# kentchen831213/-Distributed-Machine-Learning-System

Hardware: AMD Instinct MI355X
Metric: images/sec (whole node) + p50 query latency, ResNet18 bs=400 at 1/2/4/8 GPU (higher is better)
Workload: dtype fp32; 1 GPU; model=resnet18, global_batch=400, image_hw=224, batch_per_gpu=400, parallelism=dp1, graph=True, fp32_impl=split, dry_run=False

## Files before the change

### -distributed-machine-learning-system_amd/csrc/bindings.cpp

```cpp
#include <ATen/hip/HIPContext.h>
#include <torch/extension.h>

#include <mutex>

#include "kernels.h"
#include "launch_util.h"
#include "runtime/jpeg_entropy.h"

using namespace idunno;

static hipStream_t cur_stream() { return at::hip::getCurrentHIPStream().stream(); }

static void check_launch(const char* what) {
  const hipError_t e = hipGetLastError();
  TORCH_CHECK(e == hipSuccess, what, ": HIP launch failed: ", hipGetErrorString(e));
}

static torch::Tensor zero_buffer(const torch::Device& dev) {
  static std::mutex mu;
  static std::vector<torch::Tensor>* bufs = new std::vector<torch::Tensor>(64);
  const int i = dev.index() < 0 ? 0 : dev.index();
  TORCH_CHECK(i < 64, "device index out of range");
  std::lock_guard<std::mutex> lk(mu);
  auto& b = (*bufs)[i];
// ... 590 lines not shown
  TORCH_CHECK(conv3x3_band_launch(reinterpret_cast<const half_t*>(x.data_ptr()), C,
                                  reinterpret_cast<const half_t*>(w.data_ptr()), bias.data_ptr<float>(), rp, Cout,
                                  y.data_ptr(), Cout, false, B, H, W, C, Cout, relu ? 1 : 0, 1.0f, nullptr,
                                  (int)max_grid, 0, cur_stream(), true),
              "band conv: tensor too large for 32-bit buffer offsets");
  check_launch("conv3x3_band (fp16)");
  return y;
}

torch::Tensor conv2d_split(torch::Tensor x, torch::Tensor w, torch::Tensor bias, c10::optional<torch::Tensor> res,
                           int64_t KH, int64_t KW, int64_t stride, int64_t pad, bool relu, double acc_scale,
                           bool out_f32, int64_t tile, c10::optional<torch::Tensor> out, int64_t ksplit,
                           int64_t route) {
  return conv2d_split_impl(x, w, bias, res, KH, KW, stride, pad, relu, acc_scale, out_f32, tile, out, 0, false, 1.0,
                           ksplit, route);
}

torch::Tensor conv2d_split_dual(torch::Tensor x, torch::Tensor w, torch::Tensor bias, int64_t KH, int64_t KW,
                                int64_t stride, int64_t pad, bool relu, double acc_scale, double acc_scale2,
                                int64_t nsplit, bool center_only, int64_t tile) {
  TORCH_CHECK(nsplit > 0, "dual conv needs nsplit > 0");
  return conv2d_split_impl(x, w, bias, c10::nullopt, KH, KW, stride, pad, relu, acc_scale, false, tile,
                           c10::nullopt, nsplit, center_only, acc_scale2, 1, 0);
}

torch::Tensor linear_split(torch::Tensor x, torch::Tensor w, torch::Tensor bias, double acc_scale, bool relu,
                           bool out_f32, int64_t splits, int64_t tile) {
  CHECK_DEV(x);
  CHECK_DEV(w);
  CHECK_DEV(bias);
  CHECK_CONTIG(x);
  CHECK_CONTIG(w);
  CHECK_CONTIG(bias);
  CHECK_DT(x, torch::kHalf);
  CHECK_DT(w, torch::kHalf);
  CHECK_DT(bias, torch::kFloat);
  TORCH_CHECK(x.dim() == 2 && w.dim() == 2 && bias.dim() == 1, "bad ranks");
  TORCH_CHECK(w.device() == x.device() && bias.device() == x.device(), "operands on different devices");
  const int64_t M = x.size(0), K2 = x.size(1), N = w.size(0);
  TORCH_CHECK(w.size(1) == K2 && bias.size(0) == N, "shape mismatch");
  TORCH_CHECK(out_f32 ? N % 4 == 0 : N % 32 == 0, "N must be a multiple of 4 (fp32 out) / 32 (split out)");
  TORCH_CHECK(splits >= 1 && splits <= 16 && K2 % (64 * splits) == 0, "K must split into multiples of 32");
  TORCH_CHECK(splits * M * N < (1L << 31) && M * K2 < (1L << 31), "too large for int32 indexing");
  auto part = torch::empty({splits, M, N}, x.options().dtype(torch::kFloat));
  auto y = out_f32 ? torch::empty({M, N}, x.options().dtype(torch::kFloat))
                   : torch::empty({M, 2 * N}, x.options().dtype(torch::kHalf));
// ... 1066 lines not shown
  m.def("conv1x1_dual_ok", &conv1x1_dual_ok, "whether conv1x1_dual supports (K1, K2, Cout, M)");
  m.def("conv1x1_fused_next", &conv1x1_fused_next, "bottleneck tail + next block's reduce 1x1 in one pass (fp16)",
        py::arg("x1"), py::arg("x2"), py::arg("w"), py::arg("bias"), py::arg("res"), py::arg("w2"), py::arg("b2"),
        py::arg("stride"), py::arg("relu"));
  m.def("conv1x1_fused_next_ok", &conv1x1_fused_next_ok, "whether conv1x1_fused_next supports (K1, K2, N, N2, M)");
  m.def("conv1x1_dual_split", &conv1x1_dual_split, "split (fp32-accurate) form of conv1x1_dual", py::arg("x1"),
        py::arg("x2"), py::arg("w"), py::arg("bias"), py::arg("acc_scale"), py::arg("stride"), py::arg("relu"));
  m.def("conv1x1_dual_split_ok", &conv1x1_dual_split_ok, "whether conv1x1_dual_split supports (K1, K2, Cout, M)");
  m.def("conv2d_nhwc", &conv2d_nhwc, "implicit-GEMM MFMA conv + bias (+res) (+relu)", py::arg("x"), py::arg("w"),
        py::arg("bias"), py::arg("res"), py::arg("KH"), py::arg("KW"), py::arg("stride"), py::arg("pad"),
        py::arg("relu"), py::arg("out_f32") = false, py::arg("tile") = -1, py::arg("out") = py::none(),
        py::arg("ksplit") = -1, py::arg("route") = 0);
  m.def("linear_splitk", &linear_splitk, "FC layer with split-K partial GEMMs + combine", py::arg("x"),
        py::arg("w"), py::arg("bias"), py::arg("relu"), py::arg("out_f32"), py::arg("splits"), py::arg("tile") = -1);
  m.def("conv2d_split", &conv2d_split, "split-fp16 (fp32-accurate) conv: 3 f16 MFMAs per 32 channels",
        py::arg("x"), py::arg("w"), py::arg("bias"), py::arg("res"), py::arg("KH"), py::arg("KW"), py::arg("stride"),
        py::arg("pad"), py::arg("relu"), py::arg("acc_scale"), py::arg("out_f32") = false, py::arg("tile") = -1,
        py::arg("out") = py::none(), py::arg("ksplit") = -1, py::arg("route") = 0);
  m.def("conv2d_split_dual", &conv2d_split_dual,
        "two split convs of one input in one launch (downsample as the centre tap of the 3x3/s conv)",
        py::arg("x"), py::arg("w"), py::arg("bias"), py::arg("KH"), py::arg("KW"), py::arg("stride"), py::arg("pad"),
        py::arg("relu"), py::arg("acc_scale"), py::arg("acc_scale2"), py::arg("nsplit"), py::arg("center_only"),
        py::arg("tile") = -1);
  m.def("conv2d_pack3_split", &conv2d_pack3_split, "split-fp16 RGB stem conv on packed rows, fp32 out",
        py::arg("x3"), py::arg("w"), py::arg("bias"), py::arg("W"), py::arg("KH"), py::arg("KW"), py::arg("stride"),
        py::arg("pad"), py::arg("relu"), py::arg("acc_scale"), py::arg("tile") = -1);
  m.def("preprocess_pack3_split", &preprocess_pack3_split, "uint8 HWC -> split-fp16 packed-row stem input",
        py::arg("img"), py::arg("KW"), py::arg("stride"), py::arg("pad"), py::arg("start") = py::none(),
        py::arg("batch") = -1, py::arg("start_offset") = 0, py::arg("window") = -1, py::arg("sub") = 0);
  m.def("stem_u8_f16", &stem_u8_f16, "fp16 fused ResNet stem in exact-u8 form (pack_stem_split weights)",
        py::arg("img"), py::arg("w"), py::arg("bias"), py::arg("psum"), py::arg("acc_scale"), py::arg("start") = py::none(),
        py::arg("batch") = -1, py::arg("start_offset") = 0, py::arg("window") = -1, py::arg("sub") = 0);
  m.def("stem_split", &stem_split, "fp32-accurate fused split-fp16 ResNet stem (normalise+conv7x7/2+relu+maxpool)",
        py::arg("img"), py::arg("w"), py::arg("bias"), py::arg("psum"), py::arg("acc_scale"), py::arg("start") = py::none(),
        py::arg("batch") = -1, py::arg("start_offset") = 0, py::arg("window") = -1, py::arg("sub") = 0);
  m.def("linear_split", &linear_split, "fp32-accurate FC on split fp16, split-K in one launch + combine",
        py::arg("x"), py::arg("w"), py::arg("bias"), py::arg("acc_scale"), py::arg("relu"), py::arg("out_f32"),
        py::arg("splits"), py::arg("tile") = -1);
  m.def("conv3x3_band_split", &conv3x3_band_split,
        "band-staged split 3x3/s1/p1 conv (tile 70) with a persistent-grid cap (0: one workgroup per CU)",
        py::arg("x"), py::arg("w"), py::arg("bias"), py::arg("res") = py::none(), py::arg("relu") = true,
        py::arg("acc_scale") = 1.0, py::arg("out_f32") = false, py::arg("max_grid") = 0, py::arg("flags") = 0);
  m.def("conv3x3_band_f16", &conv3x3_band_f16,
        "band-staged fp16 3x3/s1/p1 conv (tile 70) with a persistent-grid cap (0: one workgroup per CU)",
        py::arg("x"), py::arg("w"), py::arg("bias"), py::arg("res"), py::arg("relu"), py::arg("max_grid") = 0);
  m.def("conv3x3_band_tiles", &conv3x3_band_tiles, "band conv tile count for (B, W, Cout)");
// ... 82 lines not shown
```

### -distributed-machine-learning-system_amd/csrc/kernels.h

```cpp
#pragma once
#include "common.h"

namespace idunno {

struct ConvArgs {
  const half_t* x;
  const half_t* w;
  const float* bias;
  const half_t* res;
  void* y;
  int B, H, W, C;
  int Ho, Wo, Cout, ldy;
  int KH, KW, stride, pad;
  int M;
  int nK;
  int cblk;
  int nsub;
  int Kpad;
  int relu;
  int tiles_n;
  int tiles_m;
  const void* zero;
  int ldx;
  int nc, wp, cpk;
  int ksplit;
  int kslice;
  long ysplit;
  float acc_scale;
  int* ovf;
  int nsplit_n;
  int center_only;
  float acc_scale2;
  int ldr;
  int kstage;
};

struct ConvF32Args {
  const float* x;
  const float* w;
  const float* bias;
  const float* res;
  float* y;
  int B, H, W, C;
  int Ho, Wo, Cout, ldy;
  int KH, KW, stride, pad;
  int M;
  int nK;
  int cblk;
  int nsub;
  int Kpad;
  int relu;
  int tiles_n, tiles_m;
  const void* zero;
  int ldx;
  int nc, wp, cpk;
  int ksplit;
  int kslice;
// ... 28 lines not shown
                                 long long sub, hipStream_t st);
void preprocess_pack3_f16_launch(const uint8_t* img, half_t* out, int B, int H, int W, int pad, int nc, int wp,
                                 const long long* start_idx, long long start_off, long long max_start,
                                 long long sub, hipStream_t st);
void preprocess_pack3_split_launch(const uint8_t* img, half_t* out, int B, int H, int W, int pad, int nc, int wp,
                                   const long long* start_idx, long long start_off, long long max_start,
                                   long long sub, hipStream_t st);
void preprocess_f32_launch(const uint8_t* img, float* out, long npix, const long long* start_idx,
                           long long start_off, long long max_start, long long sub, long pix_per_img,
                           hipStream_t st);
void maxpool_f32_launch(const float* x, float* y, int B, int H, int W, int C, int Ho, int Wo, int k, int s,
                        int pad, hipStream_t st);
void avgpool_f32_launch(const float* x, float* y, int B, int HW, int C, hipStream_t st);
void split_from_f32_launch(const float* x, half_t* y, long npix, int C, int* ovf, hipStream_t st);
void f32_from_split_launch(const half_t* x, float* y, long npix, int C, hipStream_t st);
void maxpool_split_launch(const void* x, bool in_split, half_t* y, int B, int H, int W, int C, int Ho, int Wo, int k,
                          int s, int pad, int* ovf, hipStream_t st);

void conv_igemm_launch(ConvArgs a, bool small, bool out_f32, int tile, hipStream_t st);
int conv_pick_tile(int M, int Cout);
bool conv_glds_launch(ConvArgs a, bool out_f32, int tile, hipStream_t st);
bool conv_glds_split_launch(ConvArgs a, bool out_f32, int tile, hipStream_t st);
int conv_glds_split_pick(int M, int Cout);
int conv_split_ksplit(int M, int Cout, int tile, int nk_total, int force, bool legacy = false);
bool conv1x1_small_m(long M);
void splitk_reduce_res_launch(const float* part, int S, long MN, int N, const float* bias, const half_t* res,
                              int ldr, int relu, void* y, int ldy, int fmt, int* ovf, hipStream_t st);
int conv_f16_ksplit(int M, int Cout, int tile, int nk_total, int force);
bool conv1x1_stream_supported(int C, int Cout, long M);
bool conv1x1_stream_launch(const half_t* x, const half_t* w, const float* bias, const half_t* res, half_t* y,
                           const void* zero, int M, int C, int Cout, int relu, int H, int W, int Wo, int HWo,
                           int stride, hipStream_t st);
bool conv1x1_stream_default(int C, int stride, long M);
bool conv1x1_stream_split_supported(int C, int Cout, long M);
bool conv1x1_stream_split_launch(const half_t* x, const half_t* w, const float* bias, const half_t* res, half_t* y,
                                 const void* zero, int M, int C, int Cout, int relu, float acc_scale, int* ovf, int H,
                                 int W, int Wo, int HWo, int stride, hipStream_t st);
bool conv1x1_dual_supported(int K1, int K2, int Cout, long M);
bool conv1x1_dual_launch(const half_t* x1, const half_t* x2, const half_t* w, const float* bias, half_t* y,
                         const void* zero, int M, int K1, int K2, int Cout, int relu, int H, int W, int Wo, int HWo,
                         int stride, hipStream_t st);
bool conv1x1_dual_split_supported(int K1, int K2, int Cout, long M);
bool conv1x1_dual_split_launch(const half_t* x1, const half_t* x2, const half_t* w, const float* bias, half_t* y,
                               const void* zero, int M, int K1, int K2, int Cout, int relu, float acc_scale, int* ovf,
                               int H, int W, int Wo, int HWo, int stride, hipStream_t st);
bool conv1x1_fused_next_supported(int K1, int K2, int N, int N2, long M);
// ... 81 lines not shown
```

### -distributed-machine-learning-system_amd/csrc/kernels/conv_glds.hip

```cpp
#include "../kernels.h"
#include "../launch_util.h"

namespace idunno {

typedef __attribute__((address_space(3))) void lds_void_t;
typedef __attribute__((address_space(1))) void glb_void_t;


template <int N>
__device__ __forceinline__ void wait_vmcnt() {
  static_assert(N >= 0 && N < 64, "vmcnt range");
  asm volatile("s_waitcnt vmcnt(%0)" ::"n"(N) : "memory");
}

template <int G, int NS>
__device__ __forceinline__ void wait_stages(int pending_stages) {
  if constexpr (NS >= 4) {
    if (pending_stages >= 2) { wait_vmcnt<2 * G>(); return; }
  }
  if constexpr (NS >= 3) {
    if (pending_stages >= 1) { wait_vmcnt<G>(); return; }
  }
  wait_vmcnt<0>();
}

template <int BN, int BM, int BK, int WN, int WM, int NS, bool HAS_RES, bool OUT_F32, bool P3 = false,
          bool SPLIT = false, bool KS = false>
__global__ void __launch_bounds__(64 * WN * WM, (BM % 64 != 0 && WN * WM == 8) ? 4 : 1)
conv_glds_kernel(const ConvArgs a) {
  static_assert(!SPLIT || BK == 64, "split stages are 32 channels x (hi, lo)");
  static_assert(!KS || (OUT_F32 && !HAS_RES && !P3), "split-K writes fp32 partials");
  constexpr int NW = WN * WM;
  constexpr int NT = 64 * NW;
  constexpr int TN = BN / WN, TM = BM / WM;
  constexpr int FN = TN / 16, FM = TM / 16;
  constexpr int CPR = BK / 8;
  constexpr int RB = BK * 2;
  constexpr int RPI = 64 / CPR;
  constexpr int BMD = (BM + RPI * NW - 1) / (RPI * NW) * (RPI * NW);
  constexpr int A_INS = BN / RPI, B_INS = BMD / RPI;
  static_assert(A_INS % NW == 0 && B_INS % NW == 0, "DMA instructions must split evenly over waves");
  constexpr int GA = A_INS / NW, GB = B_INS / NW, G = GA + GB;
  constexpr int A_BYTES = BN * RB, STAGE = (BN + BMD) * RB;
  static_assert(NS >= 2 && NS <= 4, "ring depth");
  static_assert(G * (NS - 2) < 64, "vmcnt immediate");

  extern __shared__ __attribute__((aligned(16))) char smem[];
  const int tid = threadIdx.x, lane = tid & 63;
  const int wave = __builtin_amdgcn_readfirstlane(tid >> 6);
  const int wn = wave / WM, wm = wave % WM;

  const int nwg = a.tiles_n * a.tiles_m;
  const int nsplit = a.ksplit > 1 ? a.ksplit : 1;
  const int lid_all = xcd_remap(blockIdx.x, nwg * nsplit);
// ... 50 lines not shown
    i_kh = a.KH / 2;
    i_kw = a.KW / 2;
    i_s = (i_kh * a.KW + i_kw) * a.cblk;
    nK = a.cblk;
  }
  if constexpr (KS) {
    i_s = split * a.kstage;
    i_cb = i_s % a.cblk;
    const int tap = i_s / a.cblk;
    i_kw = tap % a.KW;
    i_kh = tap / a.KW;
    nK = a.kstage;
  }
  constexpr uint32_t OOR = 0x80000000u;
  const auto w_rsrc = __builtin_amdgcn_make_buffer_rsrc((void*)win, 0, 0x7fffffff, 0x00020000);
  const auto x_rsrc = __builtin_amdgcn_make_buffer_rsrc((void*)xin, 0, 0x7fffffff, 0x00020000);
  uint32_t a_voff[GA], b_voff[GB];
#pragma unroll
  for (int j = 0; j < GA; ++j) {
    const int n = n0 + (wave + NW * j) * RPI + lrow;
    a_voff[j] = n < a.Cout ? (uint32_t)((n * a.Kpad + a_ch[j]) * 2) : OOR;
  }
  auto set_tap = [&]() {
#pragma unroll
    for (int j = 0; j < GB; ++j) {
      const int ih = b_ih0[j] + i_kh, iw = b_iw0[j] + i_kw;
      const bool ok = (unsigned)ih < (unsigned)a.H && (unsigned)iw < (unsigned)a.W;
      b_voff[j] = ok ? (uint32_t)((b_base[j] + (ih * a.W + iw) * ldx) * 2) : OOR;
    }
  };
  if constexpr (KS) {
    if (i_cb != 0) set_tap();
  }
  auto issue_buf = [&](int buf) {
    char* base = smem + buf * STAGE;
    if (i_cb == 0) set_tap();
    const int koff = i_s * BK * 2, coff = i_cb * BK * 2;
#pragma unroll
    for (int j = 0; j < GA; ++j)
      dma_buf16(w_rsrc, base + (wave + NW * j) * 1024, a_voff[j], koff);
#pragma unroll
    for (int j = 0; j < GB; ++j) {
      if constexpr (BMD != BM) {
        static_assert(BMD == BM || (NS == 2 && BM % RPI == 0), "skipped padding instructions need vmcnt(0) waits");
        if ((wave + NW * j) * RPI >= BM) continue;
      }
      dma_buf16(x_rsrc, base + A_BYTES + (wave + NW * j) * 1024, b_voff[j], coff);
    }
    ++i_s;
    if (++i_cb == a.cblk) {
      i_cb = 0;
      if (++i_kw == a.KW) {
        i_kw = 0;
        ++i_kh;
      }
    }
  };
  auto issue_glb = [&](int buf) {
    char* base = smem + buf * STAGE;
    const int koff = i_s * BK;
#pragma unroll
    for (int j = 0; j < GA; ++j) {
      const half_t* src = a_src[j] ? a_src[j] + koff : zero;
      __builtin_amdgcn_global_load_lds((glb_void_t*)src, (lds_void_t*)(base + (wave + NW * j) * 1024), 16, 0, 0);
    }
    const int coff = i_cb * BK;
#pragma unroll
    for (int j = 0; j < GB; ++j) {
      if constexpr (P3) {
        int q, poff = 0;
        if constexpr (SPLIT) {
          const int cc = b_ch[j] / 8;
          q = i_s * 4 + (cc & 3);
// ... 233 lines not shown
      if constexpr (OUT_F32) {
        *reinterpret_cast<float4v*>(static_cast<float*>(a.y) + (size_t)split * a.ysplit + (size_t)m * a.ldy + n) = v;
      } else if constexpr (SPLIT) {
        split_guard(a.ovf, v);
        half4v h, l;
        split_f16x4(v, h, l);
        const int q = lane >> 4;
        half_t* yp = static_cast<half_t*>(a.y) + (size_t)m * a.ldy + split_off_q(n - 4 * q, q);
        *reinterpret_cast<u32x4_sw*>(yp) = split_swap_out(h, l);
      } else {
        half4v o;
        o[0] = (half_t)v[0];
        o[1] = (half_t)v[1];
        o[2] = (half_t)v[2];
        o[3] = (half_t)v[3];
        *reinterpret_cast<half4v*>(static_cast<half_t*>(a.y) + (size_t)m * a.ldy + n) = o;
      }
    }
  }
}

static bool glds_fits(const ConvArgs& a) {
  const long xb = (long)a.B * a.H * a.W * (a.ldx ? a.ldx : a.C) * 2, wb = (long)a.Cout * a.Kpad * 2;
  return xb < (1L << 31) && wb < (1L << 31);
}

template <int BN, int BM, int BK, int WN, int WM, int NS, bool HAS_RES, bool OUT_F32, bool P3 = false,
          bool SPLIT = false, bool KS = false>
static void glds_cfg(ConvArgs a, hipStream_t st) {
  a.tiles_n = (a.Cout + BN - 1) / BN;
  a.tiles_m = (a.M + BM - 1) / BM;
  if (P3) {
    a.cblk = 1;
    const int cps = SPLIT ? BK / 16 : BK / 8;
    a.nK = (a.KH * a.cpk + cps - 1) / cps;
  } else {
    a.cblk = a.C / BK;
    a.nK = a.KH * a.KW * a.cblk;
  }
  const int grid = a.tiles_n * a.tiles_m * (a.ksplit > 1 ? a.ksplit : 1);
  constexpr int RPI_ = 64 / (BK / 8), NW_ = WN * WM;
  constexpr int BMD = (BM + RPI_ * NW_ - 1) / (RPI_ * NW_) * (RPI_ * NW_);
  const size_t lds = (size_t)NS * (BN + BMD) * BK * 2;
  auto kern = conv_glds_kernel<BN, BM, BK, WN, WM, NS, HAS_RES, OUT_F32, P3, SPLIT, KS>;
  ensure_lds_attr(reinterpret_cast<const void*>(kern), (int)lds);
  hipLaunchKernelGGL(kern, dim3(grid), dim3(64 * WN * WM), lds, st, a);
}

template <bool R, bool F>
static bool glds_dispatch(ConvArgs a, int tile, hipStream_t st) {
  switch (tile) {
    case 10: glds_cfg<128, 128, 64, 2, 2, 3, R, F>(a, st); return true;
    case 11: glds_cfg<128, 128, 32, 2, 2, 4, R, F>(a, st); return true;
    case 12: glds_cfg<64, 256, 64, 1, 4, 3, R, F>(a, st); return true;
    case 13: glds_cfg<64, 256, 32, 1, 4, 4, R, F>(a, st); return true;
    case 14: glds_cfg<128, 256, 64, 2, 4, 3, R, F>(a, st); return true;
    case 15: glds_cfg<64, 128, 64, 1, 4, 3, R, F>(a, st); return true;
    case 16: glds_cfg<128, 64, 64, 2, 2, 3, R, F>(a, st); return true;
    case 17: glds_cfg<256, 128, 64, 4, 2, 3, R, F>(a, st); return true;
    case 18: glds_cfg<128, 128, 32, 2, 2, 3, R, F>(a, st); return true;
    case 19: glds_cfg<128, 64, 32, 2, 2, 4, R, F>(a, st); return true;
    case 20: glds_cfg<64, 128, 32, 1, 4, 4, R, F>(a, st); return true;
    case 21: glds_cfg<256, 128, 32, 4, 2, 4, R, F>(a, st); return true;
    case 22: glds_cfg<128, 256, 32, 2, 4, 4, R, F>(a, st); return true;
    case 23: glds_cfg<64, 64, 64, 2, 2, 3, R, F>(a, st); return true;
    case 24: glds_cfg<128, 128, 64, 2, 4, 3, R, F>(a, st); return true;
    case 25: glds_cfg<256, 128, 64, 4, 2, 2, R, F>(a, st); return true;
// ... 39 lines not shown
}

template <bool R, bool F>
static bool glds_dispatch_split(ConvArgs a, int tile, hipStream_t st) {
  switch (tile) {
    case 26: glds_cfg<128, 128, 64, 2, 2, 2, R, F, false, true>(a, st); return true;
    case 27: glds_cfg<64, 128, 64, 1, 4, 2, R, F, false, true>(a, st); return true;
    case 34: glds_cfg<128, 64, 64, 2, 2, 2, R, F, false, true>(a, st); return true;
    case 36: glds_cfg<128, 128, 64, 2, 4, 2, R, F, false, true>(a, st); return true;
    case 38: glds_cfg<128, 64, 64, 2, 4, 2, R, F, false, true>(a, st); return true;
    case 42: glds_cfg<128, 160, 64, 4, 2, 2, R, F, false, true>(a, st); return true;
    default: return false;
  }
}

bool conv_glds_split_launch(ConvArgs a, bool out_f32, int tile, hipStream_t st) {
  if (!glds_fits(a)) return false;
  if (a.kstage > 0) return out_f32 && a.res == nullptr && glds_dispatch_ks<true>(a, tile, st);
  const bool res = a.res != nullptr;
  if (res) return out_f32 ? glds_dispatch_split<true, true>(a, tile, st) : glds_dispatch_split<true, false>(a, tile, st);
  return out_f32 ? glds_dispatch_split<false, true>(a, tile, st) : glds_dispatch_split<false, false>(a, tile, st);
}

static void ks_tile_dims(int tile, int& bn, int& bm) {
  switch (tile) {
    case 42: bn = 128; bm = 160; return;
    case 27: bn = 64; bm = 128; return;
    default: bn = 128; bm = 128; return;
  }
}
static int ksplit_rule(int force, int M, int Cout, int tile, int nk_total, long target_blocks, int min_stages) {
  if (tile != 27 && tile != 36 && tile != 42) return 1;
  if (force == 0 || force == 1) return 1;
  if (force > 1) return nk_total % force == 0 ? force : 1;
  if (nk_total < 2 * min_stages) return 1;
  int bn, bm;
  ks_tile_dims(tile, bn, bm);
  const long blocks = (long)((M + bm - 1) / bm) * ((Cout + bn - 1) / bn);
  int s = 1;
  while (s < 8 && blocks * s * 2 <= target_blocks && nk_total % (s * 2) == 0 && nk_total / (s * 2) >= min_stages)
    s *= 2;
  return s;
}
int conv_split_ksplit(int M, int Cout, int tile, int nk_total, int force, bool legacy) {
  if (legacy) return ksplit_rule(force, M, Cout, tile, nk_total, 2L * device_cu_count(), 4);
  return ksplit_rule(force, M, Cout, tile, nk_total, (long)device_cu_count(), 8);
}
int conv_f16_ksplit(int M, int Cout, int tile, int nk_total, int force) {
  return ksplit_rule(force, M, Cout, tile, nk_total, 2L * device_cu_count(), 4);
}

int conv_glds_split_pick(int M, int Cout) {
  if (Cout % 128 == 0) return M >= 50000 ? 36 : 42;
  return 27;
}

bool conv1x1_small_m(long M) { return M < 16384; }

bool conv_glds_split_p3_launch(ConvArgs a, int tile, hipStream_t st) {
  if (a.res != nullptr || a.cpk <= 0) return false;
  switch (tile) {
    case 23: glds_cfg<64, 64, 64, 2, 2, 3, false, true, true, true>(a, st); return true;
    case 27: glds_cfg<64, 128, 64, 1, 4, 2, false, true, true, true>(a, st); return true;
    case 33: glds_cfg<64, 256, 64, 1, 4, 2, false, true, true, true>(a, st); return true;
    case 35: glds_cfg<64, 64, 64, 2, 2, 2, false, true, true, true>(a, st); return true;
    case 37: glds_cfg<64, 128, 64, 1, 8, 2, false, true, true, true>(a, st); return true;
    default: return false;
  }
}

bool conv_glds_launch(ConvArgs a, bool out_f32, int tile, hipStream_t st) {
  const bool res = a.res != nullptr;
  if (a.cpk > 0) {
    if (res) return false;
    return out_f32 ? glds_dispatch_p3<true>(a, tile, st) : glds_dispatch_p3<false>(a, tile, st);
  }
  if (!glds_fits(a)) return false;
  if (a.kstage > 0) return out_f32 && !res && glds_dispatch_ks<false>(a, tile, st);
  if (res) return out_f32 ? glds_dispatch<true, true>(a, tile, st) : glds_dispatch<true, false>(a, tile, st);
// ... 10 lines not shown
```

### -distributed-machine-learning-system_amd/models/packed.py

```python
from __future__ import annotations

import contextlib
import math
import os
import threading
from dataclasses import dataclass, field

import torch
import torch.nn as nn
import torch.nn.functional as F

from . import reference as ref


@dataclass
class Conv:
    w: torch.Tensor
    b: torch.Tensor
    cin: int
    cout: int
    kh: int
    kw: int
    stride: int
    pad: int
# ... 144 lines not shown

SPLIT_BLOCK = 32


def split_eligible(cin: int, cout: int) -> bool:
    return cin % SPLIT_BLOCK == 0 and cout % SPLIT_BLOCK == 0


def to_split(x: torch.Tensor) -> torch.Tensor:
    c = x.shape[-1]
    x = x.float()
    hi = x.half()
    lo = (x - hi.float()).half()
    blk = (*x.shape[:-1], c // SPLIT_BLOCK, 1, SPLIT_BLOCK)
    return torch.cat([hi.reshape(blk), lo.reshape(blk)], dim=-2).reshape(*x.shape[:-1], 2 * c)


def from_split(xs: torch.Tensor) -> torch.Tensor:
    c = xs.shape[-1] // 2
    v = xs.float().reshape(*xs.shape[:-1], c // SPLIT_BLOCK, 2, SPLIT_BLOCK)
    return (v[..., 0, :] + v[..., 1, :]).reshape(*xs.shape[:-1], c)


def pack_split_weight(w: torch.Tensor) -> tuple[torch.Tensor, float]:
    cout, cin, kh, kw = w.shape
    if cin % SPLIT_BLOCK:
        raise ValueError(f"split weights need Cin % {SPLIT_BLOCK} == 0, got {cin}")
    e = _split_scale(w)
    ws = w.double().permute(0, 2, 3, 1) * (2.0 ** e)
    hi = ws.half()
    lo = (ws - hi.double()).half()
    blk = (cout, kh, kw, cin // SPLIT_BLOCK, 1, SPLIT_BLOCK)
    packed = torch.cat([hi.reshape(blk), lo.reshape(blk)], dim=4).reshape(cout, kh * kw * 2 * cin)
    return packed.contiguous(), 2.0 ** -e


def _split_scale(w: torch.Tensor) -> int:
    mx = float(w.abs().max())
    return 0 if mx == 0.0 else 14 - math.ceil(math.log2(mx))


def pack_split_weight_p3(w: torch.Tensor) -> tuple[torch.Tensor, float]:
    cout, cin, kh, kw = w.shape
    if cin != 3 or kw < 5:
        raise ValueError("packed-row stems take 3 input channels and KW >= 5")
    cpk = (3 * kw + 7) // 8
    k = kh * cpk * 8
    nk = (k + 31) // 32
    rows = torch.zeros(cout, kh, 8 * cpk, dtype=torch.float64)
    rows[:, :, :3 * kw] = w.double().permute(0, 2, 3, 1).reshape(cout, kh, 3 * kw)
    flat = torch.zeros(cout, nk * 32, dtype=torch.float64)
    flat[:, :k] = rows.reshape(cout, -1)
    e = _split_scale(w)
    flat = flat * (2.0 ** e)
    hi = flat.half()
    lo = (flat - hi.double()).half()
    packed = torch.cat([hi.reshape(cout, nk, 1, 32), lo.reshape(cout, nk, 1, 32)], dim=2).reshape(cout, nk * 64)
    return packed.contiguous(), 2.0 ** -e


def pack_stem_split(w: torch.Tensor, b: torch.Tensor | None = None):
    cout, cin, kh, kw = w.shape
# ... 212 lines not shown
class HipRunner:

    def __init__(self, program: Program, device=None, fuse_stem: bool = True, front_split: int | None = None,
                 winograd: bool = True, wino_variant: int | None = None, pack3: bool = True):
        from .. import ops

        ops.load()
        self.ops = ops
        self.fuse_stem = fuse_stem
        self.winograd = winograd
        self.pack3 = pack3
        self.pack3_f16 = False
        self.side_down = False
        self.stem_parts: int | None = None
        self.split = True
        self.split_front: int | None = None
        self.split_streams: int | None = None
        self._side: dict = {}
        self.wino_variant = wino_variant
        self.front_split = front_split
        self.batch_parts: int | None = None
        self.fuse_down = False
        self._dual: dict = {}
        self.fuse_down_1x1 = True
        self._dual1: dict = {}
        self.fuse_next_1x1 = True
        self.stem_u8 = False
        self.route = 0
        self.device = torch.device(device or "cuda")
        self.p = program.to(self.device)
        self._graphs: dict[int, tuple] = {}
        self.graph_pool = None
        self._ovf = torch.zeros(1, dtype=torch.int32, device=self.device)
        self.overflow_fallback = True
        self.overflow_reruns = 0
        self._capturing = False
        self.direct_launch = os.environ.get("IDUNNO_DIRECT_LAUNCH", "0") == "1"

    def _guarded(self) -> bool:
        return self.p.dtype == "fp32" and self.split and self._split_ok()

    def logits(self, img_u8: torch.Tensor, start: torch.Tensor | None = None, batch: int = -1,
               start_offset: int = 0) -> torch.Tensor:
        if not self._guarded():
            return self._logits(img_u8, start, batch, start_offset)
        self._ovf.zero_()
# ... 259 lines not shown
                    idt = self._conv(blk.down, x)
                x.record_stream(side)
                idt.record_stream(cur)
                join = side
            else:
                idt = self._conv(blk.down, x)
        y = x
        for c in blk.convs[:-1]:
            y = self._conv(c, y)
        if join is not None:
            torch.cuda.current_stream(x.device).wait_stream(join)
        return self._conv(blk.convs[-1], y, residual=idt, out=out)

    def _capture_key(self, batch: int, packed=None, slot: int = 0):
        return ((batch if slot == 0 else (batch, slot)) if packed is None else ("pk", batch, packed.data_ptr()),
                self._variant())

    def has_graph(self, batch: int, packed=None, slot: int = 0) -> bool:
        return self._capture_key(batch, packed, slot) in self._graphs

    def _variant(self) -> tuple:
        return (self.split, self.split_front, self.split_streams, self.winograd, self.wino_variant, self.pack3,
                self.pack3_f16, self.side_down, self.stem_parts, self.front_split, self.fuse_stem, self.batch_parts,
                self.fuse_down, self.fuse_down_1x1, self.fuse_next_1x1, self.stem_u8, self.route)

    def _split_ok(self) -> bool:
        p = self.p
        if p.kind == "alexnet":
            return all(v.sw is not None for k, v in p.features[1:] if k == "conv") and \
                all(f.sw is not None for f in p.fcs)
        return all(c.sw is not None for b in p.blocks for c in [*b.convs, *([b.down] if b.down else [])])

    def _alexnet_split(self, first, img_u8, start, batch, start_offset):
        o, p = self.ops, self.p
        feats = p.features[1:]
        if self.fuse_stem and first.fs is not None and first.kh == 11 and first.relu and feats \
                and feats[0][0] == "pool" and tuple(feats[0][1]) == (3, 2, 0):
            x = o.alex_stem_split(img_u8, first.fs, first.fs_bias, first.fs_psum, first.fs_scale, start, batch,
                                  start_offset)
            feats = feats[1:]
        else:
            x = self._stem_f32(first, img_u8, start, batch, start_offset)
        for k, v in feats:
            x = self._conv_split(v, x) if k == "conv" else o.maxpool2d_split(x, *v)
        x = x.reshape(x.shape[0], -1)
        for i, fc in enumerate(p.fcs):
            x = o.linear_split(x, fc.sw, fc.b, fc.s_scale, relu=fc.relu, out_f32=i == len(p.fcs) - 1)
# ... 9 lines not shown
                and c0.pad == 1 and d.kh == 1 and d.kw == 1 and d.pad == 0 and d.stride == c0.stride
                and d.cin == c0.cin and d.cout == c0.cout and c0.relu and not d.relu
                and c0.sw is not None and d.sw is not None and c0.cout % 32 == 0)

    def _dual_weights(self, blk):
        key = id(blk)
        got = self._dual.get(key)
        if got is None:
            c0, d = blk.convs[0], blk.down
            c2 = c0.sw.shape[1] // 9
            w = torch.zeros((2 * c0.cout, c0.sw.shape[1]), dtype=c0.sw.dtype, device=c0.sw.device)
            w[:c0.cout] = c0.sw
            w[c0.cout:, 4 * c2:5 * c2] = d.sw
            got = self._dual[key] = (w, torch.cat([c0.b, d.b]).contiguous())
        return got

    def _block_split(self, blk, x, last: bool = False, out=None):
        if self._dual_ok(blk):
            c0, d = blk.convs[0], blk.down
            w, b = self._dual_weights(blk)
            both = self.ops.conv2d_split_dual(x, w, b, c0.s_scale, d.s_scale, c0.cout, 3, 3, c0.stride, 1, True)
            y, idt = both[..., :2 * c0.cout], both[..., 2 * c0.cout:]
            return self._conv_split(blk.convs[1], y, residual=idt, out_f32=last, out=out)
        if not last and out is None and self._dual1_split_ok(blk, x):
            y = x
            for c in blk.convs[:-1]:
                y = self._conv_split(c, y)
            w, b, scale = self._dual1_split_weights(blk)
            return self.ops.conv1x1_dual_split(y, x, w, b, scale, blk.down.stride, blk.convs[-1].relu)
        idt = x if blk.down is None else self._conv_split(blk.down, x)
        y = x
        for c in blk.convs[:-1]:
            y = self._conv_split(c, y)
        return self._conv_split(blk.convs[-1], y, residual=idt, out_f32=last, out=out)

    def _dual1_split_ok(self, blk, x) -> bool:
        d, last = blk.down, blk.convs[-1]
        if not (self.fuse_down_1x1 and d is not None and x.is_cuda and last.sw is not None and d.sw is not None):
            return False
        if not (last.kh == last.kw == 1 and last.stride == 1 and last.pad == 0 and d.kh == d.kw == 1 and d.pad == 0):
            return False
        ho = (x.shape[1] - 1) // d.stride + 1
        return bool(self.ops.load().conv1x1_dual_split_ok(last.cin, d.cin, last.cout, x.shape[0] * ho * ho))

    def _dual1_split_weights(self, blk):
        key = ("split", id(blk))
        if key not in self._dual1:
            last, d = blk.convs[-1], blk.down
            w = torch.cat([unpack_split_weight(last).cpu(), unpack_split_weight(d).cpu()], 1)
            sw, scale = pack_split_weight(w)
            self._dual1[key] = (sw.to(self.device), (last.b + d.b).contiguous(), scale)
        return self._dual1[key]

    def _split_part(self, img_u8, start, nb, start_offset, window, sub):
        o, p, s = self.ops, self.p, self.p.stem
        if start is not None:
            x = o.stem_split(img_u8, s.fs, s.fs_bias, s.fs_psum, s.fs_scale, start, nb, start_offset,
# ... 216 lines not shown
```

### -distributed-machine-learning-system_amd/ops/__init__.py

```python
from __future__ import annotations

from ._ext import available, load, so_path

__all__ = [
    "available", "load", "so_path", "conv2d", "linear", "preprocess", "resize_crop", "resize_crop_geometry",
    "maxpool2d", "global_avgpool", "softmax_top1", "pick_tile", "pick_tile_f32", "synth_images", "stem_fused",
    "conv2d_wino", "wino_supported", "preprocess_pack3", "conv2d_pack3",
    "conv1x1_dual", "conv1x1_dual_split", "conv1x1_fused_next", "conv2d_split", "linear_split", "stem_split", "stem_u8_f16", "alex_stem_split", "alex_stem_u8_f16", "preprocess_pack3_split", "conv2d_pack3_split", "split_from_f32", "f32_from_split", "maxpool2d_split", "pick_tile_split",
    "jpeg_parse", "jpeg_entropy_batch", "jpeg_plan", "jpeg_idct", "jpeg_resize_crop",
]


def conv2d_split(x, w, bias, acc_scale: float, kh: int, kw: int, stride: int, pad: int, relu: bool,
                 residual=None, out_f32: bool = False, tile: int = -1, out=None, ksplit: int = -1, route: int = 0):
    return load().conv2d_split(x, w, bias, residual, kh, kw, stride, pad, relu, acc_scale, out_f32, tile, out,
                               ksplit, route)


def conv2d_split_dual(x, w, bias, acc_scale: float, acc_scale2: float, nsplit: int, kh: int, kw: int,
                      stride: int, pad: int, relu: bool, center_only: bool = True, tile: int = -1):
    return load().conv2d_split_dual(x, w, bias, kh, kw, stride, pad, relu, acc_scale, acc_scale2, nsplit,
                                    center_only, tile)


def preprocess_pack3_split(img_u8, kw: int, stride: int, pad: int, start=None, batch: int = -1,
                           start_offset: int = 0, window: int = -1, sub: int = 0):
    return load().preprocess_pack3_split(img_u8, kw, stride, pad, start, batch, start_offset, window, sub)


def conv2d_pack3_split(x3, w, bias, acc_scale: float, width: int, kh: int, kw: int, stride: int, pad: int,
                       relu: bool, tile: int = -1):
    return load().conv2d_pack3_split(x3, w, bias, width, kh, kw, stride, pad, relu, acc_scale, tile)


def stem_split(img_u8, w, bias, psum, acc_scale: float, start=None, batch: int = -1, start_offset: int = 0,
               window: int = -1, sub: int = 0):
    return load().stem_split(img_u8, w, bias, psum, acc_scale, start, batch, start_offset, window, sub)


def alex_stem_split(img_u8, w, bias, psum, acc_scale: float, start=None, batch: int = -1, start_offset: int = 0,
                    window: int = -1, sub: int = 0):
    return load().alex_stem_split(img_u8, w, bias, psum, acc_scale, start, batch, start_offset, window, sub)


def alex_stem_u8_f16(img_u8, w, bias, psum, acc_scale: float, start=None, batch: int = -1, start_offset: int = 0,
# ... 190 lines not shown
```

Measured before the change: 101,100 images/sec.

## Fuse downsample 1x1 conv into block's second 3x3 conv via concatenated-K GEMM

Adds a TAIL variant of the split-fp16 implicit-GEMM conv kernel that appends the strided 1x1 downsample conv of the block input as extra K steps after the 3x3 taps. The residual-projection conv and its separate tensor write and read are folded into the second conv of downsampling basic blocks, using a shared split scale and summed bias. The fused path is on by default (mode 1) for blocks that are not the last and do not use split-K. It adds a longer K loop, per-step buffer-descriptor switching, and a different rounding order from one shared weight scale.

Result: faster. 104,100 images/sec (median of 6 runs) (+2.9%).

```diff
diff --git a/-distributed-machine-learning-system_amd/csrc/bindings.cpp b/-distributed-machine-learning-system_amd/csrc/bindings.cpp
--- a/-distributed-machine-learning-system_amd/csrc/bindings.cpp
+++ b/-distributed-machine-learning-system_amd/csrc/bindings.cpp
@@ -636,6 +636,63 @@
   TORCH_CHECK(nsplit > 0, "dual conv needs nsplit > 0");
   return conv2d_split_impl(x, w, bias, c10::nullopt, KH, KW, stride, pad, relu, acc_scale, false, tile,
                            c10::nullopt, nsplit, center_only, acc_scale2, 1, 0);
+}
+
+torch::Tensor conv2d_split_tail(torch::Tensor y, torch::Tensor x2, torch::Tensor w, torch::Tensor bias,
+                                double acc_scale, int64_t stride2, bool relu, int64_t tile) {
+  CHECK_DEV(y);
+  CHECK_DEV(x2);
+  CHECK_DEV(w);
+  CHECK_DEV(bias);
+  CHECK_CONTIG(w);
+  CHECK_CONTIG(bias);
+  CHECK_DT(y, torch::kHalf);
+  CHECK_DT(x2, torch::kHalf);
+  CHECK_DT(w, torch::kHalf);
+  CHECK_DT(bias, torch::kFloat);
+  const int64_t yP = nhwc_pixel_stride(y, "y"), xP = nhwc_pixel_stride(x2, "x2");
+  TORCH_CHECK(w.dim() == 2 && bias.dim() == 1, "bad ranks");
+  TORCH_CHECK(x2.device() == y.device() && w.device() == y.device() && bias.device() == y.device(),
+              "operands on different devices");
+  const int B = y.size(0), Ho = y.size(1), Wo = y.size(2), C2 = y.size(3);
+  const int H2 = x2.size(1), W2 = x2.size(2), Cx2 = x2.size(3), Cout = w.size(0);
+  TORCH_CHECK(C2 % 64 == 0 && Cx2 % 64 == 0 && Cx2 > 0, "split operands need 2C halfs with C % 32 == 0");
+  TORCH_CHECK(w.size(1) == 9 * (int64_t)C2 + Cx2, "tail weight must be [Cout, 9*2C + 2Cx]");
+  TORCH_CHECK(bias.size(0) == Cout && Cout % 32 == 0, "bias/Cout mismatch, or Cout % 32 != 0");
+  TORCH_CHECK(stride2 >= 1 && x2.size(0) == B && Ho == (H2 - 1) / stride2 + 1 && Wo == (W2 - 1) / stride2 + 1,
+              "x2 geometry does not give y's [B, Ho, Wo] at this stride");
+  const long M = (long)B * Ho * Wo;
+  TORCH_CHECK(M * yP < (1L << 31) && (long)B * H2 * W2 * xP < (1L << 31) && M * 2 * Cout < (1L << 31),
+              "tensor too large for int32 indexing");
+  auto out = torch::empty({B, Ho, Wo, 2 * (int64_t)Cout}, y.options());
+  if (M == 0) return out;
+  ConvArgs a{};
+  a.x = reinterpret_cast<const half_t*>(y.data_ptr());
+  a.w = reinterpret_cast<const half_t*>(w.data_ptr());
+  a.bias = bias.data_ptr<float>();
+  a.y = out.data_ptr();
+  a.B = B; a.H = Ho; a.W = Wo; a.C = C2;
+  a.Ho = Ho; a.Wo = Wo; a.Cout = Cout; a.ldy = 2 * Cout;
+  a.KH = 3; a.KW = 3; a.stride = 1; a.pad = 1;
+  a.M = (int)M;
+  a.Kpad = (int)w.size(1);
+  a.relu = relu ? 1 : 0;
+  a.acc_scale = (float)acc_scale;
+  a.ovf = split_guard_for(y.device());
+  a.ldx = yP != C2 ? (int)yP : 0;
+  a.zero = zero_buffer(y.device()).data_ptr();
+  a.x2 = reinterpret_cast<const half_t*>(x2.data_ptr());
+  a.H2 = H2; a.W2 = W2; a.ldx2 = (int)xP; a.stride2 = (int)stride2;
+  a.cblk2 = Cx2 / 64;
+  const int t = tile >= 0 ? (int)tile : conv_glds_split_tail_pick(a.M, Cout);
+  TORCH_CHECK(conv_glds_split_tail_launch(a, t, cur_stream()), "conv2d_split_tail: tile ", t,
+              " has no K-tail form (36 / 42)");
+  check_launch("conv_glds_split (K tail)");
+  return out;
+}
+
+bool conv2d_split_tail_ok(int64_t B, int64_t Ho, int64_t Wo, int64_t C, int64_t Cx, int64_t Cout, int64_t mode) {
+  return conv_split_tail_default((int)B, (int)Ho, (int)Wo, (int)C, (int)Cx, (int)Cout, (int)mode);
 }
 
 torch::Tensor linear_split(torch::Tensor x, torch::Tensor w, torch::Tensor bias, double acc_scale, bool relu,
@@ -1748,6 +1805,13 @@
         py::arg("x"), py::arg("w"), py::arg("bias"), py::arg("KH"), py::arg("KW"), py::arg("stride"), py::arg("pad"),
         py::arg("relu"), py::arg("acc_scale"), py::arg("acc_scale2"), py::arg("nsplit"), py::arg("center_only"),
         py::arg("tile") = -1);
+  m.def("conv2d_split_tail", &conv2d_split_tail,
+        "split 3x3/s1/p1 conv of y + 1x1/stride2 conv of x2 as one GEMM over the concatenated K (block tail + downsample)",
+        py::arg("y"), py::arg("x2"), py::arg("w"), py::arg("bias"), py::arg("acc_scale"), py::arg("stride2"),
+        py::arg("relu"), py::arg("tile") = -1);
+  m.def("conv2d_split_tail_ok", &conv2d_split_tail_ok,
+        "whether the K-tail fusion is the default for (B, Ho, Wo, C, Cx, Cout); mode 2: wherever supported, 3: not over the band kernel",
+        py::arg("B"), py::arg("Ho"), py::arg("Wo"), py::arg("C"), py::arg("Cx"), py::arg("Cout"), py::arg("mode") = 1);
   m.def("conv2d_pack3_split", &conv2d_pack3_split, "split-fp16 RGB stem conv on packed rows, fp32 out",
         py::arg("x3"), py::arg("w"), py::arg("bias"), py::arg("W"), py::arg("KH"), py::arg("KW"), py::arg("stride"),
         py::arg("pad"), py::arg("relu"), py::arg("acc_scale"), py::arg("tile") = -1);
diff --git a/-distributed-machine-learning-system_amd/csrc/kernels.h b/-distributed-machine-learning-system_amd/csrc/kernels.h
--- a/-distributed-machine-learning-system_amd/csrc/kernels.h
+++ b/-distributed-machine-learning-system_amd/csrc/kernels.h
@@ -33,6 +33,11 @@
   float acc_scale2;
   int ldr;
   int kstage;
+  const half_t* x2;
+  int H2, W2;
+  int ldx2;
+  int stride2;
+  int cblk2;
 };
 
 struct ConvF32Args {
@@ -107,6 +112,9 @@
 bool conv_glds_launch(ConvArgs a, bool out_f32, int tile, hipStream_t st);
 bool conv_glds_split_launch(ConvArgs a, bool out_f32, int tile, hipStream_t st);
 int conv_glds_split_pick(int M, int Cout);
+bool conv_glds_split_tail_launch(ConvArgs a, int tile, hipStream_t st);
+int conv_glds_split_tail_pick(int M, int Cout);
+bool conv_split_tail_default(int B, int Ho, int Wo, int C, int Cx, int Cout, int mode = 1);
 int conv_split_ksplit(int M, int Cout, int tile, int nk_total, int force, bool legacy = false);
 bool conv1x1_small_m(long M);
 void splitk_reduce_res_launch(const float* part, int S, long MN, int N, const float* bias, const half_t* res,
diff --git a/-distributed-machine-learning-system_amd/csrc/kernels/conv_glds.hip b/-distributed-machine-learning-system_amd/csrc/kernels/conv_glds.hip
--- a/-distributed-machine-learning-system_amd/csrc/kernels/conv_glds.hip
+++ b/-distributed-machine-learning-system_amd/csrc/kernels/conv_glds.hip
@@ -25,11 +25,12 @@
 }
 
 template <int BN, int BM, int BK, int WN, int WM, int NS, bool HAS_RES, bool OUT_F32, bool P3 = false,
-          bool SPLIT = false, bool KS = false>
+          bool SPLIT = false, bool KS = false, bool TAIL = false>
 __global__ void __launch_bounds__(64 * WN * WM, (BM % 64 != 0 && WN * WM == 8) ? 4 : 1)
 conv_glds_kernel(const ConvArgs a) {
   static_assert(!SPLIT || BK == 64, "split stages are 32 channels x (hi, lo)");
   static_assert(!KS || (OUT_F32 && !HAS_RES && !P3), "split-K writes fp32 partials");
+  static_assert(!TAIL || (SPLIT && !KS && !P3 && !HAS_RES && !OUT_F32), "K tail: split in, split out, no residual");
   constexpr int NW = WN * WM;
   constexpr int NT = 64 * NW;
   constexpr int TN = BN / WN, TM = BM / WM;
@@ -126,6 +127,25 @@
     a_voff[j] = n < a.Cout ? (uint32_t)((n * a.Kpad + a_ch[j]) * 2) : OOR;
   }
   auto set_tap = [&]() {
+    if constexpr (TAIL) {
+      if (i_kh == a.KH) {
+#pragma unroll
+        for (int j = 0; j < GB; ++j) {
+          const int row = (wave + NW * j) * RPI + lrow;
+          const int m = m0 + row;
+          uint32_t v = OOR;
+          if (row < BM && m < a.M) {
+            const int hw = a.Ho * a.Wo;
+            const int b = m / hw, r = m - b * hw;
+            const int oh = r / a.Wo, ow = r - oh * a.Wo;
+            const int pix = (b * a.H2 + oh * a.stride2) * a.W2 + ow * a.stride2;
+            v = (uint32_t)((pix * a.ldx2 + (lslot ^ swz_r(row, CPR)) * 8) * 2);
+          }
+          b_voff[j] = v;
+        }
+        return;
+      }
+    }
 #pragma unroll
     for (int j = 0; j < GB; ++j) {
       const int ih = b_ih0[j] + i_kh, iw = b_iw0[j] + i_kw;
@@ -140,6 +160,12 @@
     char* base = smem + buf * STAGE;
     if (i_cb == 0) set_tap();
     const int koff = i_s * BK * 2, coff = i_cb * BK * 2;
+    const auto b_rsrc = [&] {
+      if constexpr (TAIL)
+        return __builtin_amdgcn_make_buffer_rsrc((void*)(i_kh == a.KH ? a.x2 : xin), 0, 0x7fffffff, 0x00020000);
+      else
+        return x_rsrc;
+    }();
 #pragma unroll
     for (int j = 0; j < GA; ++j)
       dma_buf16(w_rsrc, base + (wave + NW * j) * 1024, a_voff[j], koff);
@@ -149,10 +175,10 @@
         static_assert(BMD == BM || (NS == 2 && BM % RPI == 0), "skipped padding instructions need vmcnt(0) waits");
         if ((wave + NW * j) * RPI >= BM) continue;
       }
-      dma_buf16(x_rsrc, base + A_BYTES + (wave + NW * j) * 1024, b_voff[j], coff);
+      dma_buf16(b_rsrc, base + A_BYTES + (wave + NW * j) * 1024, b_voff[j], coff);
     }
     ++i_s;
-    if (++i_cb == a.cblk) {
+    if (++i_cb == (TAIL && i_kh == a.KH ? a.cblk2 : a.cblk)) {
       i_cb = 0;
       if (++i_kw == a.KW) {
         i_kw = 0;
@@ -432,11 +458,12 @@
 
 static bool glds_fits(const ConvArgs& a) {
   const long xb = (long)a.B * a.H * a.W * (a.ldx ? a.ldx : a.C) * 2, wb = (long)a.Cout * a.Kpad * 2;
-  return xb < (1L << 31) && wb < (1L << 31);
+  const long x2b = a.x2 ? (long)a.B * a.H2 * a.W2 * a.ldx2 * 2 : 0;
+  return xb < (1L << 31) && wb < (1L << 31) && x2b < (1L << 31);
 }
 
 template <int BN, int BM, int BK, int WN, int WM, int NS, bool HAS_RES, bool OUT_F32, bool P3 = false,
-          bool SPLIT = false, bool KS = false>
+          bool SPLIT = false, bool KS = false, bool TAIL = false>
 static void glds_cfg(ConvArgs a, hipStream_t st) {
   a.tiles_n = (a.Cout + BN - 1) / BN;
   a.tiles_m = (a.M + BM - 1) / BM;
@@ -446,13 +473,13 @@
     a.nK = (a.KH * a.cpk + cps - 1) / cps;
   } else {
     a.cblk = a.C / BK;
-    a.nK = a.KH * a.KW * a.cblk;
+    a.nK = a.KH * a.KW * a.cblk + (TAIL ? a.cblk2 : 0);
   }
   const int grid = a.tiles_n * a.tiles_m * (a.ksplit > 1 ? a.ksplit : 1);
   constexpr int RPI_ = 64 / (BK / 8), NW_ = WN * WM;
   constexpr int BMD = (BM + RPI_ * NW_ - 1) / (RPI_ * NW_) * (RPI_ * NW_);
   const size_t lds = (size_t)NS * (BN + BMD) * BK * 2;
-  auto kern = conv_glds_kernel<BN, BM, BK, WN, WM, NS, HAS_RES, OUT_F32, P3, SPLIT, KS>;
+  auto kern = conv_glds_kernel<BN, BM, BK, WN, WM, NS, HAS_RES, OUT_F32, P3, SPLIT, KS, TAIL>;
   ensure_lds_attr(reinterpret_cast<const void*>(kern), (int)lds);
   hipLaunchKernelGGL(kern, dim3(grid), dim3(64 * WN * WM), lds, st, a);
 }
@@ -538,6 +565,16 @@
   return out_f32 ? glds_dispatch_split<false, true>(a, tile, st) : glds_dispatch_split<false, false>(a, tile, st);
 }
 
+bool conv_glds_split_tail_launch(ConvArgs a, int tile, hipStream_t st) {
+  if (a.x2 == nullptr || a.cblk2 <= 0 || a.res != nullptr || a.kstage > 0 || a.ksplit > 1 || a.nsplit_n > 0) return false;
+  if (!glds_fits(a)) return false;
+  switch (tile) {
+    case 36: glds_cfg<128, 128, 64, 2, 4, 2, false, false, false, true, false, true>(a, st); return true;
+    case 42: glds_cfg<128, 160, 64, 4, 2, 2, false, false, false, true, false, true>(a, st); return true;
+    default: return false;
+  }
+}
+
 static void ks_tile_dims(int tile, int& bn, int& bm) {
   switch (tile) {
     case 42: bn = 128; bm = 160; return;
@@ -571,6 +608,22 @@
   return 27;
 }
 
+int conv_glds_split_tail_pick(int M, int Cout) {
+  const int t = conv_glds_split_pick(M, Cout);
+  return t == 42 ? 42 : 36;
+}
+
+bool conv_split_tail_default(int B, int Ho, int Wo, int C, int Cx, int Cout, int mode) {
+  if (mode <= 0) return false;
+  if (B <= 0 || C % 32 != 0 || Cx % 32 != 0 || Cx <= 0 || Cout % 128 != 0) return false;
+  const long M = (long)B * Ho * Wo;
+  if (4 * M * (C > Cout ? C : Cout) >= (1L << 31) || 16 * M * Cx >= (1L << 31)) return false;
+  if (mode == 2) return true;
+  if (conv_split_ksplit((int)M, Cout, conv_glds_split_pick((int)M, Cout), 9 * (C / 32), -1) > 1) return false;
+  if (mode == 3) return !(Ho == Wo && conv3x3_band_supported(Ho, Wo, C, Cout) && conv3x3_band_default(B, Wo, Cout));
+  return true;
+}
+
 bool conv1x1_small_m(long M) { return M < 16384; }
 
 bool conv_glds_split_p3_launch(ConvArgs a, int tile, hipStream_t st) {
diff --git a/-distributed-machine-learning-system_amd/models/packed.py b/-distributed-machine-learning-system_amd/models/packed.py
--- a/-distributed-machine-learning-system_amd/models/packed.py
+++ b/-distributed-machine-learning-system_amd/models/packed.py
@@ -190,11 +190,12 @@
     return (v[..., 0, :] + v[..., 1, :]).reshape(*xs.shape[:-1], c)
 
 
-def pack_split_weight(w: torch.Tensor) -> tuple[torch.Tensor, float]:
+def pack_split_weight(w: torch.Tensor, e: int | None = None) -> tuple[torch.Tensor, float]:
     cout, cin, kh, kw = w.shape
     if cin % SPLIT_BLOCK:
         raise ValueError(f"split weights need Cin % {SPLIT_BLOCK} == 0, got {cin}")
-    e = _split_scale(w)
+    if e is None:
+        e = _split_scale(w)
     ws = w.double().permute(0, 2, 3, 1) * (2.0 ** e)
     hi = ws.half()
     lo = (ws - hi.double()).half()
@@ -206,6 +207,15 @@
 def _split_scale(w: torch.Tensor) -> int:
     mx = float(w.abs().max())
     return 0 if mx == 0.0 else 14 - math.ceil(math.log2(mx))
+
+
+def pack_split_tail_weight(w2: torch.Tensor, wd: torch.Tensor) -> tuple[torch.Tensor, float]:
+    if wd.shape[0] != w2.shape[0] or tuple(wd.shape[2:]) != (1, 1) or tuple(w2.shape[2:]) != (3, 3):
+        raise ValueError("tail weights: [Cout, C, 3, 3] and [Cout, Cx, 1, 1]")
+    e = _split_scale(torch.cat([w2.flatten(), wd.flatten()]))
+    s2, scale = pack_split_weight(w2, e)
+    sd, _ = pack_split_weight(wd, e)
+    return torch.cat([s2, sd], dim=1).contiguous(), scale
 
 
 def pack_split_weight_p3(w: torch.Tensor) -> tuple[torch.Tensor, float]:
@@ -464,6 +474,8 @@
         self.batch_parts: int | None = None
         self.fuse_down = False
         self._dual: dict = {}
+        self.fuse_down_tail = 1
+        self._tail: dict = {}
         self.fuse_down_1x1 = True
         self._dual1: dict = {}
         self.fuse_next_1x1 = True
@@ -769,7 +781,8 @@
     def _variant(self) -> tuple:
         return (self.split, self.split_front, self.split_streams, self.winograd, self.wino_variant, self.pack3,
                 self.pack3_f16, self.side_down, self.stem_parts, self.front_split, self.fuse_stem, self.batch_parts,
-                self.fuse_down, self.fuse_down_1x1, self.fuse_next_1x1, self.stem_u8, self.route)
+                self.fuse_down, self.fuse_down_1x1, self.fuse_next_1x1, self.stem_u8, self.route,
+                int(self.fuse_down_tail))
 
     def _split_ok(self) -> bool:
         p = self.p
@@ -825,6 +838,11 @@
             both = self.ops.conv2d_split_dual(x, w, b, c0.s_scale, d.s_scale, c0.cout, 3, 3, c0.stride, 1, True)
             y, idt = both[..., :2 * c0.cout], both[..., 2 * c0.cout:]
             return self._conv_split(blk.convs[1], y, residual=idt, out_f32=last, out=out)
+        if not last and out is None and self._tail_ok(blk, x):
+            c0, c1, d = blk.convs[0], blk.convs[1], blk.down
+            y = self._conv_split(c0, x)
+            w, b, scale = self._tail_weights(blk)
+            return self.ops.conv2d_split_tail(y, x, w, b, scale, d.stride, c1.relu)
         if not last and out is None and self._dual1_split_ok(blk, x):
             y = x
             for c in blk.convs[:-1]:
@@ -836,6 +854,29 @@
         for c in blk.convs[:-1]:
             y = self._conv_split(c, y)
         return self._conv_split(blk.convs[-1], y, residual=idt, out_f32=last, out=out)
+
+    def _tail_ok(self, blk, x) -> bool:
+        d = blk.down
+        if not (int(self.fuse_down_tail) and d is not None and len(blk.convs) == 2 and x.is_cuda):
+            return False
+        c0, c1 = blk.convs
+        if not (c1.kh == c1.kw == 3 and c1.stride == 1 and c1.pad == 1 and d.kh == d.kw == 1 and d.pad == 0
+                and not d.relu and d.cout == c1.cout and c1.cin == c0.cout and d.cin == c0.cin
+                and c1.sw is not None and d.sw is not None and c0.sw is not None):
+            return False
+        ho = (x.shape[1] + 2 * c0.pad - c0.kh) // c0.stride + 1
+        wo = (x.shape[2] + 2 * c0.pad - c0.kw) // c0.stride + 1
+        if ho != (x.shape[1] - 1) // d.stride + 1 or wo != (x.shape[2] - 1) // d.stride + 1:
+            return False
+        return self.ops.conv2d_split_tail_ok(x.shape[0], ho, wo, c1.cin, d.cin, c1.cout, int(self.fuse_down_tail))
+
+    def _tail_weights(self, blk):
+        key = id(blk)
+        if key not in self._tail:
+            c1, d = blk.convs[1], blk.down
+            sw, scale = pack_split_tail_weight(unpack_split_weight(c1).cpu(), unpack_split_weight(d).cpu())
+            self._tail[key] = (sw.to(self.device), (c1.b + d.b).contiguous(), scale)
+        return self._tail[key]
 
     def _dual1_split_ok(self, blk, x) -> bool:
         d, last = blk.down, blk.convs[-1]
diff --git a/-distributed-machine-learning-system_amd/ops/__init__.py b/-distributed-machine-learning-system_amd/ops/__init__.py
--- a/-distributed-machine-learning-system_amd/ops/__init__.py
+++ b/-distributed-machine-learning-system_amd/ops/__init__.py
@@ -6,7 +6,7 @@
     "available", "load", "so_path", "conv2d", "linear", "preprocess", "resize_crop", "resize_crop_geometry",
     "maxpool2d", "global_avgpool", "softmax_top1", "pick_tile", "pick_tile_f32", "synth_images", "stem_fused",
     "conv2d_wino", "wino_supported", "preprocess_pack3", "conv2d_pack3",
-    "conv1x1_dual", "conv1x1_dual_split", "conv1x1_fused_next", "conv2d_split", "linear_split", "stem_split", "stem_u8_f16", "alex_stem_split", "alex_stem_u8_f16", "preprocess_pack3_split", "conv2d_pack3_split", "split_from_f32", "f32_from_split", "maxpool2d_split", "pick_tile_split",
+    "conv1x1_dual", "conv1x1_dual_split", "conv1x1_fused_next", "conv2d_split", "conv2d_split_tail", "conv2d_split_tail_ok", "linear_split", "stem_split", "stem_u8_f16", "alex_stem_split", "alex_stem_u8_f16", "preprocess_pack3_split", "conv2d_pack3_split", "split_from_f32", "f32_from_split", "maxpool2d_split", "pick_tile_split",
     "jpeg_parse", "jpeg_entropy_batch", "jpeg_plan", "jpeg_idct", "jpeg_resize_crop",
 ]
 
@@ -21,6 +21,14 @@
                       stride: int, pad: int, relu: bool, center_only: bool = True, tile: int = -1):
     return load().conv2d_split_dual(x, w, bias, kh, kw, stride, pad, relu, acc_scale, acc_scale2, nsplit,
                                     center_only, tile)
+
+
+def conv2d_split_tail(y, x2, w, bias, acc_scale: float, stride2: int, relu: bool, tile: int = -1):
+    return load().conv2d_split_tail(y, x2, w, bias, acc_scale, stride2, relu, tile)
+
+
+def conv2d_split_tail_ok(b: int, ho: int, wo: int, c: int, cx: int, cout: int, mode: int = 1) -> bool:
+    return bool(load().conv2d_split_tail_ok(b, ho, wo, c, cx, cout, mode))
 
 
 def preprocess_pack3_split(img_u8, kw: int, stride: int, pad: int, start=None, batch: int = -1,
```
